# iPERDance/iPERCore

Hardware: AMD Instinct MI355X
Metric: synthesized frames/sec at 512x512 (run_imitator) (higher is better)
Workload: dtype f32; 1 GPU; run_imitator 512x512 single src/ref pair, 300-frame reference clip frame-sharded over 1 GPU(s), AttLWB-SPADE generator fp32 (BASELINE configs[1] at N = 1, configs[2] at N = 8); poses=imitate, image_size=512, frame_batch=300, frame_batch_requested=384, world_size=1, parallelism=frame-shard x1, batches_in_flight=1, weights=random-init (seeded) of the real architecture, 36,276,992 params

## Files before the change

### ipercore_amd/csrc/conv_winograd4.hip

```cpp
#include <hip/hip_runtime.h>
#include "lwg_common.h"
#include "lwg_conv_wino.h"

#define W4_THREADS 512
#define W4_PBX 8
#define W4_PBY 4
#define W4_NB 64
#define W4_KS 8
#define W4_HW 34
#define W4_HH 18
#ifndef W4_RS
#define W4_RS 40
#endif
#define W4_PLANE (18 * W4_RS + 4)
#define W4_RAW (W4_KS * W4_PLANE)
#define W4_VS (36 * W4_KS * 32)
#define W4_NEL (W4_HW * W4_HH * 2)
#define W4_NQ 3
#define W4_DUMP_OFF (2 * W4_RAW + 2 * W4_VS)
#define W4_DUMP (W4_THREADS + 3 * W4_PLANE)
#define W4_LOOP (W4_DUMP_OFF + W4_DUMP)
#define W4_MSR 68
#define W4_NPL 28
#define W4_MS (W4_NPL * 16 * W4_MSR)
#define W4_BIAS_OFF (W4_LOOP > W4_MS ? W4_LOOP : W4_MS)
#define W4F_SLOT(s) (((s) / CW4F_NSX) * CW4F_HH * W4_RS + ((s) % CW4F_NSX) * (W4_RS / CW4F_NSX))
#define W4F_PLANE (CW4F_NS / CW4F_NSX * CW4F_HH * W4_RS + 4)
static_assert(W4_RS / CW4F_NSX >= CW4F_HW && (W4_RS / CW4F_NSX) % 4 == 0 && W4F_PLANE >= W4_PLANE, "two sub-tile halo rows per LDS row");
#define W4F_LOOP (2 * W4_KS * W4F_PLANE + 2 * W4_VS + W4_THREADS + 3 * W4F_PLANE)
#define W4F_BIAS_OFF (W4F_LOOP > W4_MS ? W4F_LOOP : W4_MS)
static_assert(CW4F_SX == 16 && CW4F_SY == 8 && CW4F_NS * CW4F_ROUNDS * 64 == W4_NQ * W4_THREADS, "sub-tile halo: four slots x six wave rounds = the staged elements");
#ifndef LWG_W4_XCD
#define LWG_W4_XCD 1
#endif
#ifndef LWG_W4_CHUNK
#define LWG_W4_CHUNK 1
#endif
#ifndef LWG_W4_RDMAP
#define LWG_W4_RDMAP 1
#endif
#ifndef LWG_W4_SMALL
#define LWG_W4_SMALL 1
#endif
#define W4SB() __builtin_amdgcn_sched_barrier(0)

#ifdef LWG_W4_TS
#define W4TS(i) do { if (tid == 0 && lab_bi == 1) reinterpret_cast<unsigned long long*>(const_cast<float*>(a.res))[(size_t)blockIdx.x * 16 + (i)] = __builtin_readcyclecounter(); } while (0)
#define W4TSA(i) do { if (tid == 0) reinterpret_cast<unsigned long long*>(const_cast<float*>(a.res))[(size_t)blockIdx.x * 16 + (i)] = __builtin_readcyclecounter(); } while (0)
#else
#define W4TS(i) do { } while (0)
#define W4TSA(i) do { } while (0)
#endif

#ifndef W4_NT
#define W4_NT 0
#endif
#ifndef W4_NT_LD
#define W4_NT_LD W4_NT
#endif
#ifndef W4_NT_RES
#define W4_NT_RES 0
#endif
#ifndef W4_NT_ST
#define W4_NT_ST 2
#endif

__device__ __forceinline__ void w4_bt6(const float (&r)[6], float (&v)[6]) {
    const float a = __builtin_fmaf(-4.f, r[2], r[4]), b = __builtin_fmaf(-4.f, r[1], r[3]);
    const float c = r[4] - r[2], e = r[3] - r[1];
    v[0] = __builtin_fmaf(-5.f, r[2], __builtin_fmaf(4.f, r[0], r[4]));
    v[1] = a + b;
    v[2] = a - b;
    v[3] = __builtin_fmaf(2.f, e, c);
    v[4] = __builtin_fmaf(-2.f, e, c);
    v[5] = __builtin_fmaf(-5.f, r[3], __builtin_fmaf(4.f, r[1], r[5]));
}

__device__ __forceinline__ float w4_spade_mod(float x, float mu, float rs, float gam, float bet) { return (x - mu) * rs * (1.f + gam) + bet; }
template <int NR>
__device__ __forceinline__ void w4_act16(int act, floatx4 (&o)[NR]) {
    lwg_act_dispatch(act, [&](auto ACTC) {
        constexpr int EA = decltype(ACTC)::value;
#pragma unroll
        for (int i = 0; i < NR; ++i)
#pragma unroll
            for (int c = 0; c < 4; ++c) o[i][c] = lwg_act_c<EA>(o[i][c], act);
    });
}

template <int EPI, bool TWO, bool SM, bool LIST, bool FINE = false, bool SPLIT = false>
__device__ __forceinline__ void w4_body(const LwgConvArgs& a, const LwgConvLists& sk) {
    static_assert(!FINE || (LIST && !SM && !TWO && LWG_W4_RDMAP), "the sub-tile form: a list-driven 8-wave launch");
    static_assert(!SPLIT || (SM && !LIST && EPI == LWG_EPI_NONE), "the split form: 4-wave blocks, plain epilogue");
    constexpr int RS = W4_RS;
    constexpr int PLANE = FINE ? W4F_PLANE : W4_PLANE;
    constexpr int RAW = W4_KS * PLANE;
    constexpr int DUMP_OFF = 2 * RAW + 2 * W4_VS;
    constexpr int BIAS_OFF = FINE ? W4F_BIAS_OFF : W4_BIAS_OFF;
    constexpr bool SMS = SM && EPI == LWG_EPI_SPADE;
    constexpr int NVP = SM && !SMS ? 2 : 1;
    constexpr int NTH = SM ? 256 : W4_THREADS;
    constexpr int NQ = SM ? 5 : W4_NQ;
    constexpr int NBV = SM ? 32 : W4_NB;
    constexpr int MSR = SM ? 36 : W4_MSR;
    constexpr int NHF = SM ? 2 : 1;
    extern __shared__ __attribute__((aligned(16))) float smem[];
    const int wid = __builtin_amdgcn_readfirstlane(threadIdx.x >> 6);
    const float* __restrict__ bias = a.bias;
    const int H = a.H, W = a.W, Cin = a.C0 + a.C1, N = a.N;
    float* __restrict__ y = SPLIT ? a.y + cw4_slab_offset((int)blockIdx.z, a.M, N) : a.y;
    float* const raw0 = smem;
    float* const Ms = smem;
    const int tid = threadIdx.x, lane = tid & 63;
    const CwGrid g = cw_grid(a.B, H, W, N, 4 * W4_PBX, 4 * W4_PBY, NBV);
    const CwOrder o = cw_order(cw4_order_kind(LWG_W4_XCD, LWG_W4_CHUNK, SM, gridDim.x, N / NBV, Cin, N, g.tiles, g.total), gridDim.x, blockIdx.x, N / NBV, g);
    int blk = blockIdx.x;
    const int nall = FINE ? cw4f_in_image_total(a.B, H, W) : g.tiles;
    const int nht = LIST ? min(max(__builtin_amdgcn_readfirstlane(sk.counts[0]), 0), nall) : 0;
    const int nhe = (FINE ? cw4f_groups(nht) : nht) * (N / NBV);
    const bool lst = FINE ? true : LIST ? nht < nall : false;
    const bool run = lst ? blk < nhe : true;
    const int nst = Cin / W4_KS;
    const int sbeg = SPLIT ? cw4_slice_begin((int)blockIdx.z, a.cshift) : 0;
    const int send = SPLIT ? cw4_slice_end((int)blockIdx.z, a.cshift, nst) : nst;
    const __amdgpu_buffer_rsrc_t ru = __builtin_amdgcn_make_buffer_rsrc(const_cast<float*>(a.w), 0, (int)(144u * (unsigned)Cin * (unsigned)N), 0x00020000);
    const int q = wid & 3, ct = SM ? 0 : wid >> 2;
    const int half = SM ? 0 : wid >> 2;
    floatx16 acc[9];
    CwBlock<NQ, TWO> bk;
    unsigned uvoff, uvoffc;
    int fs0 = 0, fs1 = 0;
    auto setup = [&](int id) {
        int cb, t;
        if constexpr (FINE) {
            int tids = tid;
            asm volatile("" : "+v"(tids));
            int fsub[CW4F_NS], slot;
            cw_list_entry(id, N / NBV, slot, cb);
#pragma unroll
            for (int k = 0; k < CW4F_NS; ++k) {
                const int ix = cw4f_slot_index(slot, k, nht);
                fsub[k] = ix < 0 ? -1 : min(max(__builtin_amdgcn_readfirstlane(sk.heavy[ix]), 0), CW4F_NS * g.tiles - 1);
            }
            bk.n0 = cw_n0(cb, NBV);
            const int hs = wid >> 1, u = hs == 0 ? fsub[0] : hs == 1 ? fsub[1] : hs == 2 ? fsub[2] : fsub[3];
            int b, x0, y0;
            cw4f_corner(g, max(u, 0), b, x0, y0);
            bk.rx0 = cw_image_rsrc(a.x0, __builtin_amdgcn_readfirstlane(b), H, W, a.C0, 4u);
#pragma unroll
            for (int k = 0; k < NQ; ++k) {
                int s, j;
                cw4f_halo_elem(tids + NTH * k, s, j);
                bk.voff0[k] = cw4f_halo_voff(u >= 0, j, x0, y0, H, W, a.C0);
            }
            fs0 = (wid >> 2) ? fsub[1] : fsub[0], fs1 = (wid >> 2) ? fsub[CW4F_NSX + 1] : fsub[CW4F_NSX];
        } else if constexpr (LIST) {
            if (lst) {
                int slot;
                cw_list_entry(id, N / NBV, slot, cb);
                t = min(max(__builtin_amdgcn_readfirstlane(sk.heavy[slot]), 0), g.tiles - 1);
            } else {
                cw_block(o, id, cb, t);
            }
        } else {
            cw_block(o, id, cb, t);
        }
        if constexpr (!FINE) {
        bk.locate(a, g, t, 4 * W4_PBX, 4 * W4_PBY, SMS ? cw4_n0_spade_small(cb) : cw_n0(cb, NBV));
        int tids = tid;
        asm volatile("" : "+v"(tids));
        bk.halo(a, tids, NTH, W4_HW, W4_NEL);
        }
        const int col = SMS ? bk.n0 + (((lane & 31) >> 4) << 5) + (lane & 15) : bk.n0 + ct * 32 + (lane & 31);
        uvoff = (unsigned)(((lane >> 5) * 9 * N + 4 * col) * 4);
        uvoffc = (unsigned)(((lane >> 5) * 9 * N + 8 * N + col) * 4);
    };
    if (run) setup(blk);
    int wst[NQ];
#pragma unroll
    for (int k = 0; k < NQ; ++k) {
        const int i = tid + NTH * k;
        if constexpr (FINE) {
            int s, j, hy, hx, hq;
            cw4f_halo_elem(i, s, j);
            cw4f_halo_place(j, hy, hx, hq);
            wst[k] = j < CW4F_NEL ? 4 * hq * PLANE + W4F_SLOT(s) + hy * RS + hx : DUMP_OFF + tid;
        } else {
        const int pix = i >> 1, hq = i & 1, hy = pix / W4_HW, hx = pix - hy * W4_HW;
        wst[k] = i < W4_NEL ? 4 * hq * PLANE + hy * RS + hx : DUMP_OFF + tid;
        }
    }
    floatx4 rreg[NQ];
    auto rld1 = [&](int st, int k) -> floatx4 {
#ifdef W4_LAB_HFIX
        const int c = 0 * st;
#else
        const int c = st * W4_KS;
#endif
        return bk.template rld1<W4_NT_LD>(a, c, k);
    };
    auto rst1 = [&](int buf, int k, floatx4 v) { cw_rst1(raw0 + buf * RAW + wst[k], PLANE, v); };
    floatx4 ufa[4], ufb[4];
    float ufc[4];
    const unsigned ukk = (unsigned)N * 72u;
    const unsigned uq = (unsigned)q * (unsigned)nst * 4u * ukk;
    const unsigned ubo = (unsigned)N * 16u;
    auto uldpart = [&](int set, int st, int kk, int part) {
#ifdef W4_LAB_UFIX
        const unsigned so = uq + 0u * (unsigned)(st + kk);
#else
        const unsigned so = uq + (unsigned)(st * 4 + kk) * ukk;
#endif
        if (part == 0) ufa[set] = cw_buf_load(ru, uvoff, so);
        else if (part == 1) ufb[set] = cw_buf_load(ru, uvoff, so + ubo);
        else ufc[set] = __builtin_bit_cast(float, __builtin_amdgcn_raw_buffer_load_b32(ru, (int)uvoffc, (int)so, 0));
    };
    auto uldset = [&](int set, int st, int kk) {
#ifdef W4_LAB_UFIX
        const unsigned so = uq + 0u * (unsigned)(st + kk);
#else
        const unsigned so = uq + (unsigned)(st * 4 + kk) * ukk;
#endif
        ufa[set] = cw_buf_load(ru, uvoff, so);
        ufb[set] = cw_buf_load(ru, uvoff, so + ubo);
        ufc[set] = __builtin_bit_cast(float, __builtin_amdgcn_raw_buffer_load_b32(ru, (int)uvoffc, (int)so, 0));
    };
    const int patch = tid & 31, tc = (tid >> 5) & 7;
    const int pty = patch >> 3, ptx = patch & 7;
    int pby = pty, pbx = ptx, pslot = 0;
    if constexpr (FINE) {
        cw4f_patch_in_slot(pty, ptx, pby, pbx);
        pslot = W4F_SLOT(cw4f_slot_of_patch(pty, ptx));
    }
    unsigned dbs = (unsigned)(tc * PLANE + pslot + (4 * pby) * RS + 4 * pbx) >> 2;
    asm volatile("" : "+v"(dbs));
    dbs <<= 2;
    unsigned dbx[NHF], vbx[NHF], vbt[NHF];
    float alpha[NHF], beta[NHF], nbeta[NHF];
#pragma unroll
    for (int hi = 0; hi < NHF; ++hi) {
        const int hf = SM ? hi : half;
        dbx[hi] = (unsigned)(tc * PLANE + pslot + (4 * pby + hf) * RS + 4 * pbx) >> 2;
        asm volatile("" : "+v"(dbx[hi]));
        dbx[hi] <<= 2;
        vbx[hi] = (unsigned)(2 * RAW + (hf ? 30 : 0) * W4_KS * 32 + tc * 32 + patch);
        vbt[hi] = (unsigned)(2 * RAW + (hf ? 18 : 6) * W4_KS * 32 + tc * 32 + patch);
        asm volatile("" : "+v"(vbx[hi]));
        asm volatile("" : "+v"(vbt[hi]));
        alpha[hi] = hf ? -1.f : -4.f;
        beta[hi] = hf ? 2.f : 1.f;
        nbeta[hi] = -beta[hi];
    }
    unsigned fbs[2];
    fbs[0] = (unsigned)(2 * RAW + (6 * q) * W4_KS * 32 + lane);
    fbs[1] = (unsigned)(2 * RAW + (6 * (4 + (q >> 1)) + 3 * (q & 1)) * W4_KS * 32 + lane);
    asm volatile("" : "+v"(fbs[0]));
    asm volatile("" : "+v"(fbs[1]));
    float fb[9];
    auto frag1 = [&](int buf, int kk, int j) -> float {
        return smem[fbs[j < 6 ? 0 : 1] + buf * W4_VS + ((j < 6 ? j : j - 6) * W4_KS + 2 * kk) * 32];
// ... 99 lines not shown
                    vst6(vbt[hi], set ^ 1, step - 12, v);
                }
            }
            W4SB();
        };
        if constexpr (!SM) {
            mf(0, 0, true); ul(0, 0);
            mf(0, 1, true); halo(0);
            mf(0, 2, true); ul(0, 1); tr(0, 0);
            mf(0, 3, true); halo(1); tr(0, 1);
            mf(0, 4, true); ul(0, 2); tr(0, 2);
            mf(0, 5, true); halo(2);
            mf(0, 6, true); tr(0, 3);
            mf(0, 7, true); tr(0, 4);
            mf(0, 8, true); tr(0, 5);
            mf(1, 0, true); ul(1, 0); tr(0, 6);
            mf(1, 1, true); tr(0, 7);
            mf(1, 2, true); ul(1, 1); tr(0, 8); tr(0, 9);
            mf(1, 3, true); tr(0, 10);
            mf(1, 4, true); ul(1, 2);
            mf(1, 5, true); tr(0, 11);
            mf(1, 6, true); tr(0, 12);
            mf(1, 7, true);
            mf(1, 8, true); tr(0, 13);
            mf(2, 0, true); ul(2, 0);
            mf(2, 1, true);
            mf(2, 2, true); ul(2, 1);
            mf(2, 3, true);
            mf(2, 4, true); ul(2, 2);
            mf(2, 5, true); mf(2, 6, true); mf(2, 7, true); mf(2, 8, true);
        } else {
            mf(0, 0, true); ul(0, 0); halo(0);
            mf(0, 1, true); tr(0, 0);
            mf(0, 2, true); ul(0, 1); tr(0, 1);
            mf(0, 3, true); halo(1); tr(0, 2);
            mf(0, 4, true); ul(0, 2); tr(0, 3);
            mf(0, 5, true); halo(2); tr(0, 4);
            mf(0, 6, true); tr(0, 5);
            mf(0, 7, true); halo(3); tr(0, 6);
            mf(0, 8, true); tr(0, 7);
            mf(1, 0, true); ul(1, 0); tr(0, 8); tr(0, 9);
            mf(1, 1, true); halo(4); tr(0, 10);
            mf(1, 2, true); ul(1, 1); tr(0, 11);
            mf(1, 3, true); tr(0, 12);
            mf(1, 4, true); ul(1, 2); tr(0, 13);
            mf(1, 5, true); tr(1, 0);
            mf(1, 6, true); tr(1, 1);
            mf(1, 7, true); tr(1, 2);
            mf(1, 8, true); tr(1, 3);
            mf(2, 0, true); ul(2, 0); tr(1, 4);
            mf(2, 1, true); tr(1, 5);
            mf(2, 2, true); ul(2, 1); tr(1, 6);
            mf(2, 3, true); tr(1, 7);
            mf(2, 4, true); ul(2, 2); tr(1, 8); tr(1, 9);
            mf(2, 5, true); tr(1, 10);
            mf(2, 6, true); tr(1, 11);
            mf(2, 7, true); tr(1, 12);
            mf(2, 8, true); tr(1, 13);
        }
        __syncthreads();
        W4SB();
        mf(3, 0, nxt); ul(3, 0);
        mf(3, 1, nxt);
        mf(3, 2, nxt); ul(3, 1);
        mf(3, 3, nxt);
        mf(3, 4, nxt); ul(3, 2);
        mf(3, 5, nxt); mf(3, 6, nxt); mf(3, 7, nxt); mf(3, 8, nxt);
    };

    floatx4 r0[NQ], r1[NQ];
    float bq;
    auto issue_loads = [&]() {
        bq = bias ? bias[SMS ? bk.n0 + (((tid & 31) >> 4) << 5) + (tid & 15) : bk.n0 + (tid & (NBV - 1))] : 0.f;
#pragma unroll
        for (int k = 0; k < NQ; ++k) {
            r0[k] = rld1(sbeg, k);
            r1[k] = rld1(sbeg + 1, k);
        }
        uldset(0, sbeg, 0);
        uldset(1, sbeg, 1);
#pragma unroll
        for (int k = 0; k < NQ; ++k) rreg[k] = rld1(send - sbeg > 2 ? sbeg + 2 : sbeg + 1, k);
    };
    if (run) issue_loads();
#ifdef LWG_W4_TS
    int lab_bi = 0;
#endif
    W4TSA(11);
    if (run) for (;;) {
    W4TS(0);
#pragma unroll
    for (int k = 0; k < NQ; ++k) {
        rst1(0, k, r0[k]);
        rst1(1, k, r1[k]);
    }
    if (tid < NBV) smem[BIAS_OFF + tid] = bq;
    __syncthreads();
    transform_full(0);
    __syncthreads();
#pragma unroll
    for (int j = 0; j < 9; ++j) fb[j] = frag1(0, 0, j);
#pragma unroll
    for (int j = 0; j < 9; ++j)
#pragma unroll
        for (int r = 0; r < 16; ++r) acc[j][r] = 0.f;
    if (q == 1) {
#pragma unroll
        for (int g = 0; g < 4; ++g) {
            const floatx4 b4 = *reinterpret_cast<const floatx4*>(smem + BIAS_OFF + ct * 32 + 8 * g + 4 * (lane >> 5));
#pragma unroll
            for (int k = 0; k < 4; ++k) acc[1][4 * g + k] = b4[k];
        }
    }
    W4TS(1);
    {
        int s = sbeg;
        for (; s + 2 < send; s += 2) {
            iteration(s, IntC<0>(), IntC<1>());
            iteration(s + 1, IntC<1>(), IntC<1>());
        }
        iteration(s, IntC<0>(), IntC<1>());
        iteration(s + 1, IntC<1>(), IntC<0>());
    }
    W4TS(2);
    int eb = FINE ? 0 : bk.b, ex0 = FINE ? 0 : bk.x0, ey0 = FINE ? 0 : bk.y0;
    const int en0 = bk.n0;
    const int es0 = fs0, es1 = fs1;
#pragma unroll
    for (int r = 0; r < 16; ++r) {
        const float m0 = acc[0][r], m1 = acc[1][r], m2 = acc[2][r], m3 = acc[3][r], m4 = acc[4][r], m5 = acc[5][r];
        const float s12 = m1 + m2, d12 = m1 - m2, s34 = m3 + m4, d34 = m3 - m4;
        acc[0][r] = (m0 + s12) + s34;
        acc[1][r] = __builtin_fmaf(2.f, d34, d12);
        acc[2][r] = __builtin_fmaf(4.f, s34, s12);
        acc[3][r] = __builtin_fmaf(8.f, d34, d12) + m5;
    }
    if (q & 1) {
#pragma unroll
        for (int r = 0; r < 16; ++r) {
            const float h0 = acc[6][r], h1 = acc[7][r];
            acc[6][r] = h0 + h1;
            acc[7][r] = h0 - h1;
        }
    } else {
#pragma unroll
        for (int r = 0; r < 16; ++r) {
            const float h0 = acc[6][r], h1 = acc[7][r], h2 = acc[8][r];
            acc[6][r] = (h0 + h1) + h2;
            acc[7][r] = h1 - h2;
            acc[8][r] = h1 + h2;
        }
    }
    W4TS(4);
    int tide = tid;
    asm volatile("" : "+v"(tide));
    const int lanee = tide & 63;
    const int rb = wid & 3;
    const unsigned l5 = (unsigned)lanee & 31u, gsel = (0x0FF0F00Fu >> l5) & 1u;
    const int gidx = __builtin_popcount((gsel ? 0x0FF0F00Fu : 0xF00F0FF0u) & ((1u << l5) - 1u));
    const int p16 = LWG_W4_RDMAP && !SM ? (wid >> 2) * 4 + 2 * (lanee >> 5) + (gsel ? 0 : 1) + 8 * (gidx >> 3) : (wid >> 2) * 8 + (lanee >> 3);
    const int n4 = SMS ? (lanee & 3) * 4 : LWG_W4_RDMAP && !SM ? (gidx & 7) * 4 : (lanee & 7) * 4;
    const int cbase = SMS ? (en0 >> 6) * 32 + ((en0 >> 4) & 1) * 16 : en0 >> 1;
    floatx4 mu, rs;
    typedef unsigned int w4_u4 __attribute__((ext_vector_type(4)));
    const unsigned img_bytes = (unsigned)(H * W) * (unsigned)a.YC * 4u;
    const float* const esrc = EPI == LWG_EPI_SPADE ? a.xn : EPI == LWG_EPI_RESIDUAL ? a.res : a.y;
    __amdgpu_buffer_rsrc_t ry, re;
    auto eframe = [&]() {
        if (EPI == LWG_EPI_SPADE) {
            mu = *reinterpret_cast<const floatx4*>(a.mean + (size_t)eb * a.YC + cbase + n4);
            rs = *reinterpret_cast<const floatx4*>(a.rstd + (size_t)eb * a.YC + cbase + n4);
        }
        ry = __builtin_amdgcn_make_buffer_rsrc(y + (size_t)eb * H * W * a.YC, 0, (int)img_bytes, 0x00020000);
        re = __builtin_amdgcn_make_buffer_rsrc(const_cast<float*>(esrc) + (size_t)eb * H * W * a.YC, 0, (int)img_bytes, 0x00020000);
    };
    if constexpr (!FINE) eframe();
    const int chan = EPI == LWG_EPI_SPADE ? cbase + n4 : a.ycoff + en0 + n4;
    bool more = false;
    int nblk = blk;
#pragma unroll
    for (int ph = 0; ph < 2; ++ph) {
        if (ph == 1) __syncthreads();
        if constexpr (FINE) {
            const int u = ph ? es1 : es0;
            int ub;
            cw4f_corner(g, max(u, 0), ub, ex0, ey0);
            eb = __builtin_amdgcn_readfirstlane(ub);
            if (u < 0) ex0 = W, ey0 = H;
            eframe();
        }
        if (((lanee >> 4) & 1) == ph) {
            float* dst = Ms + (lanee & 15) * MSR + ct * 32 + 4 * (lanee >> 5);
#pragma unroll
            for (int g = 0; g < 4; ++g) {
#pragma unroll
                for (int bb = 0; bb < 4; ++bb)
                    *reinterpret_cast<floatx4*>(dst + (4 * q + bb) * 16 * MSR + 8 * g) = floatx4{acc[bb][4 * g], acc[bb][4 * g + 1], acc[bb][4 * g + 2], acc[bb][4 * g + 3]};
#pragma unroll
                for (int i = 0; i < 3; ++i)
                    *reinterpret_cast<floatx4*>(dst + (16 + 3 * q + i) * 16 * MSR + 8 * g) = floatx4{acc[6 + i][4 * g], acc[6 + i][4 * g + 1], acc[6 + i][4 * g + 2], acc[6 + i][4 * g + 3]};
            }
        }
        unsigned vo[NVP][4];
#pragma unroll
        for (int hp = 0; hp < NVP; ++hp) {
            const int p = ph * 16 + (SMS ? lanee >> 2 : SM ? 8 * hp + (lanee >> 3) : p16);
            const int ox = ex0 + 4 * (FINE ? (p & 7) % (CW4F_SX / 4) : (p & 7)) + rb, oyb = ey0 + 4 * (FINE ? (p >> 3) % (CW4F_SY / 4) : (p >> 3));
#pragma unroll
            for (int i = 0; i < 4; ++i)
                vo[hp][i] = cw4_out_voff(ox, oyb + i, H, W, a.YC, chan);
        }
        floatx4 ext[2][4];
        if (EPI != LWG_EPI_NONE) {
#pragma unroll
            for (int h = 0; h < (EPI == LWG_EPI_SPADE ? 1 : 2); ++h)
#pragma unroll
                for (int i = 0; i < 4; ++i) ext[h][i] = __builtin_bit_cast(floatx4, __builtin_amdgcn_raw_buffer_load_b128(re, (int)cw4_out_group(vo[NVP == 2 ? h : 0][i], h, !SM), 0, W4_NT_RES));
        }
        if (ph == 1) {
            W4TS(8);
            if constexpr (!SPLIT) {
            nblk = blk + (int)gridDim.x;
            if constexpr (FINE) more = nblk < nhe;
            else if constexpr (LIST) more = lst ? nblk < nhe : cw_has_block(o, nblk);
            else more = cw_has_block(o, nblk);
            setup(more ? nblk : blk);
            W4TS(9);
            issue_loads();
            W4TS(10);
            }
        }
        __syncthreads();
        if (ph == 0) W4TS(5); else W4TS(7);
        floatx4 gam[4];
#pragma unroll
        for (int h = 0; h < 2; ++h) {
            const float* base = Ms + (SMS ? lanee >> 2 : SM ? 8 * h + (lanee >> 3) : p16) * MSR + (SMS ? h * 16 : SM ? 0 : h * 32) + n4;
            floatx4 F[6];
#pragma unroll
            for (int xi = 0; xi < 4; ++xi) F[xi] = *reinterpret_cast<const floatx4*>(base + (4 * xi + rb) * 16 * MSR);
            const int ia = rb == 0 ? 0 : rb == 2 ? 2 : 1, ib = (rb & 1) ? 4 : 3;
            const float cb = (float)(1 << rb);
#pragma unroll
            for (int r = 0; r < 2; ++r) {
                const float* hb = base + (16 + 6 * r) * 16 * MSR;
                const floatx4 pa = *reinterpret_cast<const floatx4*>(hb + ia * 16 * MSR);
                const floatx4 pb = *reinterpret_cast<const floatx4*>(hb + ib * 16 * MSR);
                floatx4 f;
#pragma unroll
                for (int c = 0; c < 4; ++c) f[c] = __builtin_fmaf(cb, pb[c], pa[c]);
                if (rb == 3) f += *reinterpret_cast<const floatx4*>(hb + 5 * 16 * MSR);
                F[4 + r] = f;
            }
            floatx4 o[4];
#pragma unroll
            for (int c = 0; c < 4; ++c) {
                const float s12 = F[1][c] + F[2][c], d12 = F[1][c] - F[2][c], s34 = F[3][c] + F[4][c], d34 = F[3][c] - F[4][c];
                o[0][c] = (F[0][c] + s12) + s34;
                o[1][c] = __builtin_fmaf(2.f, d34, d12);
                o[2][c] = __builtin_fmaf(4.f, s34, s12);
                o[3][c] = __builtin_fmaf(8.f, d34, d12) + F[5][c];
            }
            if (EPI == LWG_EPI_SPADE) {
                if (h == 0) {
#pragma unroll
                    for (int i = 0; i < 4; ++i) gam[i] = o[i];
                    continue;
                }
#pragma unroll
                for (int i = 0; i < 4; ++i)
#pragma unroll
                    for (int c = 0; c < 4; ++c) o[i][c] = w4_spade_mod(ext[0][i][c], mu[c], rs[c], gam[i][c], o[i][c]);
            } else if (EPI == LWG_EPI_RESIDUAL) {
                if (a.act == LWG_ACT_RELU_MASK) {
#pragma unroll
                    for (int i = 0; i < 4; ++i)
#pragma unroll
                        for (int c = 0; c < 4; ++c) o[i][c] = ext[h][i][c] > 0.f ? o[i][c] : 0.f;
                } else {
#pragma unroll
                    for (int i = 0; i < 4; ++i) o[i] += ext[h][i];
                }
            }
            w4_act16(a.act, o);
#pragma unroll
            for (int i = 0; i < 4; ++i)
                __builtin_amdgcn_raw_buffer_store_b128(__builtin_bit_cast(w4_u4, o[i]), ry, (int)cw4_out_group(vo[NVP == 2 ? h : 0][i], h, EPI != LWG_EPI_SPADE && !SM), 0, W4_NT_ST);
        }
        if (ph == 0) W4TS(6);
    }
    W4TS(3);
#ifdef LWG_W4_TS
    ++lab_bi;
#endif
    if (!more) break;
    blk = nblk;
    __syncthreads();
    }
    W4TSA(12);
#ifdef LWG_W4_TS
    if (tid == 0) reinterpret_cast<unsigned long long*>(const_cast<float*>(a.res))[(size_t)blockIdx.x * 16 + 13] = (unsigned long long)lab_bi;
#endif
    if constexpr (LIST) {
        typedef unsigned int w4_u4 __attribute__((ext_vector_type(4)));
        constexpr int NQD = EPI == LWG_EPI_SPADE ? 8 : 16;
        constexpr int NPASS = (FINE ? CW4F_SX * CW4F_SY : 512) * NQD / W4_THREADS, NI = NPASS < 4 ? NPASS : 4;
        const int ncb = N / NBV;
        const int nend = nhe + min(max(__builtin_amdgcn_readfirstlane(sk.counts[1]), 0), nall - nht) * ncb;
        const unsigned img_bytes = (unsigned)(H * W) * (unsigned)a.YC * 4u;
        const __amdgpu_buffer_rsrc_t rc = __builtin_amdgcn_make_buffer_rsrc(const_cast<float*>(sk.cal), 0, (int)((unsigned)(H * W) * (unsigned)(EPI == LWG_EPI_SPADE ? N : a.YC) * 4u), 0x00020000);
#pragma unroll 1
        for (int id = cw_list_first_light((int)blockIdx.x, (int)gridDim.x, nhe); id < nend; id += (int)gridDim.x) {
            int slot, cb;
            cw_list_entry(id - nhe, ncb, slot, cb);
            const int t = min(max(__builtin_amdgcn_readfirstlane(sk.light[slot]), 0), (FINE ? CW4F_NS : 1) * g.tiles - 1);
            const int en0 = cw_n0(cb, NBV);
            int eb, ex0, ey0;
            if constexpr (FINE) {
                cw4f_corner(g, t, eb, ex0, ey0);
                eb = __builtin_amdgcn_readfirstlane(eb);
            } else {
                eb = __builtin_amdgcn_readfirstlane(cw_image(g, t));
                cw_corner(g, t - eb * g.bx * g.by, 4 * W4_PBX, 4 * W4_PBY, ex0, ey0);
            }
            const __amdgpu_buffer_rsrc_t ry = __builtin_amdgcn_make_buffer_rsrc(y + (size_t)eb * H * W * a.YC, 0, (int)img_bytes, 0x00020000);
            int px, py, q4;
            cw4_light_elem(tid, 0, W4_THREADS, NQD, px, py, q4);
            if constexpr (EPI == LWG_EPI_SPADE) {
                const __amdgpu_buffer_rsrc_t re = __builtin_amdgcn_make_buffer_rsrc(const_cast<float*>(a.xn) + (size_t)eb * H * W * a.YC, 0, (int)img_bytes, 0x00020000);
                const int cbase = en0 >> 1;
                const floatx4 mu = *reinterpret_cast<const floatx4*>(a.mean + (size_t)eb * a.YC + cbase + 4 * q4);
                const floatx4 rs = *reinterpret_cast<const floatx4*>(a.rstd + (size_t)eb * a.YC + cbase + 4 * q4);
#pragma unroll 1
                for (int it = 0; it < NPASS; it += NI) {
                    unsigned vo[NI];
                    floatx4 o[NI], gam[NI], xv[NI];
#pragma unroll
                    for (int i = 0; i < NI; ++i) {
                        cw4_light_elem(tid, it + i, W4_THREADS, NQD, px, py, q4);
                        if constexpr (FINE) cw4f_light_pixel(px, py);
                        vo[i] = cw4_out_voff(ex0 + px, ey0 + py, H, W, a.YC, cbase + 4 * q4);
                        const unsigned vc = cw4_out_voff(ex0 + px, ey0 + py, H, W, N, en0 + 4 * q4);
                        gam[i] = cw_buf_load(rc, cw4_out_group(vc, 0, true), 0u);
                        o[i] = cw_buf_load(rc, cw4_out_group(vc, 1, true), 0u);
                        xv[i] = cw_buf_load<W4_NT_RES>(re, vo[i], 0u);
                    }
#pragma unroll
                    for (int i = 0; i < NI; ++i)
#pragma unroll
                        for (int c = 0; c < 4; ++c) o[i][c] = w4_spade_mod(xv[i][c], mu[c], rs[c], gam[i][c], o[i][c]);
                    w4_act16(a.act, o);
#pragma unroll
                    for (int i = 0; i < NI; ++i) __builtin_amdgcn_raw_buffer_store_b128(__builtin_bit_cast(w4_u4, o[i]), ry, (int)vo[i], 0, W4_NT_ST);
                }
            } else {
#pragma unroll 1
                for (int it = 0; it < NPASS; it += NI) {
                    unsigned vo[NI];
                    floatx4 o[NI];
#pragma unroll
                    for (int i = 0; i < NI; ++i) {
                        cw4_light_elem(tid, it + i, W4_THREADS, NQD, px, py, q4);
                        if constexpr (FINE) cw4f_light_pixel(px, py);
                        vo[i] = cw4_out_voff(ex0 + px, ey0 + py, H, W, a.YC, a.ycoff + en0 + 4 * q4);
                        o[i] = cw_buf_load(rc, vo[i], 0u);
                    }
#pragma unroll
                    for (int i = 0; i < NI; ++i) __builtin_amdgcn_raw_buffer_store_b128(__builtin_bit_cast(w4_u4, o[i]), ry, (int)vo[i], 0, W4_NT_ST);
                }
            }
        }
    }
}

template <int EPI, bool TWO, bool SM = false>
__global__ __launch_bounds__(SM ? 256 : W4_THREADS, 1) void lwg_conv_winograd4_kernel(const LwgConvArgs a) {
    w4_body<EPI, TWO, SM, false>(a, LwgConvLists{});
}
template <bool TWO>
__global__ __launch_bounds__(256, 1) void lwg_conv_winograd4_split_kernel(const LwgConvArgs a) {
    w4_body<LWG_EPI_NONE, TWO, true, false, false, true>(a, LwgConvLists{});
}
template <int EPI>
__global__ __launch_bounds__(W4_THREADS, 1) void lwg_conv_winograd4_list_kernel(const LwgConvArgs a, const LwgConvLists sk) {
    w4_body<EPI, false, false, true>(a, sk);
}
template <int EPI>
__global__ __launch_bounds__(W4_THREADS, 1) void lwg_conv_winograd4_fine_kernel(const LwgConvArgs a, const LwgConvLists sk) {
    if (__builtin_amdgcn_readfirstlane(sk.counts[0]) >= cw4f_in_image_total(a.B, a.H, a.W)) return;
    w4_body<EPI, false, false, true, true>(a, sk);
}
template <int EPI>
__global__ __launch_bounds__(W4_THREADS, 1) void lwg_conv_winograd4_fine_plain_kernel(const LwgConvArgs a, const LwgConvLists sk) {
    if (__builtin_amdgcn_readfirstlane(sk.counts[0]) < cw4f_in_image_total(a.B, a.H, a.W)) return;
    w4_body<EPI, false, false, false>(a, LwgConvLists{});
}


__global__ __launch_bounds__(256) void lwg_winograd4_panel_kernel(const float* __restrict__ wp, float* __restrict__ U, int Cin, int N, LwgWinoTaps taps) {
    const int n = blockIdx.x * 64 + (threadIdx.x & 63), c = blockIdx.y * 4 + (threadIdx.x >> 6);
    if (n >= N || c >= Cin) return;
    double g[3][3];
#pragma unroll
    for (int r = 0; r < 3; ++r)
#pragma unroll
        for (int s = 0; s < 3; ++s) {
            const int k = ((c >> 5) * 9 + taps.t[3 * r + s]) * 32 + (c & 31);
            g[r][s] = (double)wp[((size_t)(k >> 2) * N + n) * 4 + (k & 3)];
        }
    const double G[6][3] = {{1.0 / 4, 0, 0}, {-1.0 / 6, -1.0 / 6, -1.0 / 6}, {-1.0 / 6, 1.0 / 6, -1.0 / 6}, {1.0 / 24, 1.0 / 12, 1.0 / 6}, {1.0 / 24, -1.0 / 12, 1.0 / 6}, {0, 0, 1}};
    double t[6][3];
#pragma unroll
    for (int i = 0; i < 6; ++i)
#pragma unroll
        for (int s = 0; s < 3; ++s) t[i][s] = G[i][0] * g[0][s] + G[i][1] * g[1][s] + G[i][2] * g[2][s];
    const int s8 = c >> 3, kk = (c & 7) >> 1, kh = c & 1;
#pragma unroll
    for (int qq = 0; qq < 4; ++qq) {
        float* dst = U + ((((size_t)qq * (Cin >> 3) + s8) * 4 + kk) * 2 + kh) * 9 * (size_t)N;
        float o[9];
#pragma unroll
        for (int j = 0; j < 9; ++j) {
            const int xi = j < 6 ? qq : 4 + (qq >> 1), nu = j < 6 ? j : 3 * (qq & 1) + (j - 6);
            o[j] = (float)(t[xi][0] * G[nu][0] + t[xi][1] * G[nu][1] + t[xi][2] * G[nu][2]);
        }
        *reinterpret_cast<floatx4*>(dst + 4 * n) = floatx4{o[0], o[1], o[2], o[3]};
        *reinterpret_cast<floatx4*>(dst + 4 * (size_t)N + 4 * n) = floatx4{o[4], o[5], o[6], o[7]};
        dst[8 * (size_t)N + n] = o[8];
    }
}

__device__ __forceinline__ double w4_panel_sum3(double a0, double b0, double a1, double b1, double a2, double b2) {
#pragma clang fp contract(off)
    const double p = a0 * b0;
    return __builtin_fma(a2, b2, __builtin_fma(a1, b1, p));
}
__device__ __forceinline__ void lwg_winograd4_panels_pair(const float* __restrict__ wp, float* __restrict__ U, int Cin, int N, const int* t9, int c, int n) {
    double g[3][3];
#pragma unroll
    for (int r = 0; r < 3; ++r)
#pragma unroll
        for (int s = 0; s < 3; ++s) {
            const int k = ((c >> 5) * 9 + t9[3 * r + s]) * 32 + (c & 31);
            g[r][s] = (double)wp[((size_t)(k >> 2) * N + n) * 4 + (k & 3)];
        }
    const double G[6][3] = {{1.0 / 4, 0, 0}, {-1.0 / 6, -1.0 / 6, -1.0 / 6}, {-1.0 / 6, 1.0 / 6, -1.0 / 6}, {1.0 / 24, 1.0 / 12, 1.0 / 6}, {1.0 / 24, -1.0 / 12, 1.0 / 6}, {0, 0, 1}};
    double t[6][3];
#pragma unroll
    for (int i = 0; i < 6; ++i)
#pragma unroll
        for (int s = 0; s < 3; ++s) t[i][s] = w4_panel_sum3(G[i][0], g[0][s], G[i][1], g[1][s], G[i][2], g[2][s]);
    const int s8 = c >> 3, kk = (c & 7) >> 1, kh = c & 1;
#pragma unroll
    for (int qq = 0; qq < 4; ++qq) {
        float* dst = U + ((((size_t)qq * (Cin >> 3) + s8) * 4 + kk) * 2 + kh) * 9 * (size_t)N;
// ... 137 lines not shown
```

### ipercore_amd/csrc/lwg_conv_wino.h

```cpp
#pragma once
#include <stddef.h>
#include "lwg_conv_args.h"

#ifdef __HIPCC__
#define CW_FN __host__ __device__ __forceinline__
#else
#define CW_FN static inline
#endif
#ifdef __HIP_DEVICE_COMPILE__
#define CW_UNIFORM(v) __builtin_amdgcn_readfirstlane(v)
#else
#define CW_UNIFORM(v) (v)
#endif
#define CW_OOB 0xC0000000u
#define CW_KS 8
#define CW_NB 64
struct CwGrid { int bx, by, tiles, total; };
CW_FN CwGrid cw_grid(int B, int H, int W, int N, int ex, int ey, int nbv) {
    const int bx = (W + ex - 1) / ex, by = (H + ey - 1) / ey, tiles = bx * by * B;
    return CwGrid{bx, by, tiles, tiles * (N / nbv)};
}
CW_FN long long cw_total_blocks(int B, int H, int W, int N, int ex, int ey, int nbv) {
    return (long long)((W + ex - 1) / ex) * ((H + ey - 1) / ey) * B * (N / nbv);
}

enum { CW_COLMAJOR = 0, CW_CHUNK = 1, CW_XCD = 2 };
struct CwOrder { int kind, nwg, wg, ncb, tiles, total, xg, xr; };

CW_FN int cw4_order_kind(int xcd_sw, int chunk_sw, bool sm, unsigned nwg, int ncb, int Cin, int N, int tiles, int total) {
    const bool xcd = xcd_sw && !sm && (nwg & 7u) == 0 && (ncb == 4 || ncb == 8 || (ncb == 2 && (Cin >= 192 || xcd_sw == 2))) && (int)nwg < total && tiles >= (int)nwg / ncb;
    return xcd ? CW_XCD : chunk_sw == 2 || (chunk_sw == 1 && 144u * (unsigned)Cin * (unsigned)N <= (5u << 20)) ? CW_CHUNK : CW_COLMAJOR;
}
CW_FN CwOrder cw_order(int kind, unsigned nwg, unsigned wg, int ncb, const CwGrid& g) {
    return CwOrder{kind, (int)nwg, (int)wg, ncb, g.tiles, g.total, (int)nwg / ncb, (int)(((wg & 7u) / (unsigned)ncb) * (nwg >> 3) + (wg >> 3))};
}
CW_FN bool cw_has_block(const CwOrder& o, int id) {
    return o.kind == CW_XCD ? (id / o.nwg) * o.xg + o.xr < o.tiles : id < o.total;
}
CW_FN void cw_block(const CwOrder& o, int id, int& cb, int& t) {
    if (o.kind == CW_XCD) {
        cb = (int)((unsigned)o.wg & 7u) & (o.ncb - 1);
        t = CW_UNIFORM((id / o.nwg) * o.xg + o.xr);
    } else if (o.kind == CW_CHUNK) {
        const int G = o.nwg, per = G * o.ncb;
        const int ch = CW_UNIFORM(id / per);
        const int r = id - ch * per, base = ch * G;
        const int nt = o.tiles - base < G ? o.tiles - base : G;
        cb = CW_UNIFORM(r / nt);
        t = CW_UNIFORM(base + r - cb * nt);
    } else {
        cb = CW_UNIFORM(id / o.tiles);
        t = CW_UNIFORM(id - cb * o.tiles);
    }
}
CW_FN int cw_image(const CwGrid& g, int t) { return t / (g.bx * g.by); }
CW_FN void cw_corner(const CwGrid& g, int t_in_image, int ex, int ey, int& x0, int& y0) { x0 = (t_in_image % g.bx) * ex, y0 = (t_in_image / g.bx) * ey; }
CW_FN int cw_n0(int cb, int nbv) { return cb * nbv; }
CW_FN int cw4_n0_spade_small(int cb) { return (cb >> 1) * 64 + (cb & 1) * 16; }
CW_FN int cw_halo_pixel(int i, int hw, int nel, int lgp, int x0, int y0, int H, int W) {
    const int pix = i >> lgp, hy = pix / hw, hx = pix - hy * hw;
    const int gy = y0 - 1 + hy, gx = x0 - 1 + hx;
    return i < nel && gy >= 0 && gy < H && gx >= 0 && gx < W ? gy * W + gx : -1;
}
CW_FN unsigned cw_halo_pixel_voff(int lin, int i, int lgp, int C, int ebytes) {
    return lin >= 0 ? (unsigned)(lin * C + (16 / ebytes) * (i & ((1 << lgp) - 1))) * (unsigned)ebytes : CW_OOB;
}
CW_FN unsigned cw_halo_voff(int i, int hw, int nel, int lgp, int x0, int y0, int H, int W, int C, int ebytes) {
    return cw_halo_pixel_voff(cw_halo_pixel(i, hw, nel, lgp, x0, y0, H, W), i, lgp, C, ebytes);
}
CW_FN bool cw_stage_second(int c, int C0, bool two) { return two && c >= C0; }
CW_FN unsigned cw_stage_soff(int c, int C0, bool two, int ebytes) { return (unsigned)(cw_stage_second(c, C0, two) ? c - C0 : c) * (unsigned)ebytes; }
CW_FN unsigned cw4_out_voff(int ox, int oy, int H, int W, int YC, int chan) {
    return ox < W && oy < H ? (unsigned)((oy * W + ox) * YC + chan) * 4u : CW_OOB;
}
CW_FN unsigned cw4_out_group(unsigned vo, int h, bool grouped) { return vo + (grouped ? 128u * (unsigned)h : 0u); }

struct CwWindow { int x0, y0, x1, y1; };
CW_FN CwWindow cw_block_window(int x0, int y0, int ex, int ey, int d, int H, int W) {
    return CwWindow{x0 - d > 0 ? x0 - d : 0, y0 - d > 0 ? y0 - d : 0, x0 + ex + d < W ? x0 + ex + d : W, y0 + ey + d < H ? y0 + ey + d : H};
}
CW_FN void cw_list_entry(int e, int ncb, int& slot, int& cb) { slot = e / ncb, cb = e - slot * ncb; }
CW_FN int cw_list_first_light(int wg, int nwg, int nhe) { return wg >= nhe ? wg : wg + (nhe - wg + nwg - 1) / nwg * nwg; }
CW_FN void cw4_light_elem(int tid, int it, int nth, int nq, int& px, int& py, int& q4) {
    const int e = it * nth + tid, p = e / nq;
    q4 = e - p * nq, px = p & 31, py = p >> 5;
}

#define CW4F_SX 16
#define CW4F_SY 8
#define CW4F_NSX (32 / CW4F_SX)
#define CW4F_NS (CW4F_NSX * (16 / CW4F_SY))
#define CW4F_HW (CW4F_SX + 2)
#define CW4F_HH (CW4F_SY + 2)
#define CW4F_NEL (CW4F_HW * CW4F_HH * 2)
#define CW4F_ROUNDS ((CW4F_NEL + 63) / 64)
CW_FN int cw4f_slot_of_patch(int pty, int ptx) { return (pty / (CW4F_SY / 4)) * CW4F_NSX + ptx / (CW4F_SX / 4); }
CW_FN void cw4f_patch_in_slot(int pty, int ptx, int& ly, int& lx) { ly = pty % (CW4F_SY / 4), lx = ptx % (CW4F_SX / 4); }
CW_FN void cw4f_corner(const CwGrid& g, int u, int& b, int& x0, int& y0) {
    const int t = u / CW4F_NS, s = u - t * CW4F_NS;
    b = cw_image(g, t);
    cw_corner(g, t - b * g.bx * g.by, 32, 16, x0, y0);
    x0 += (s % CW4F_NSX) * CW4F_SX, y0 += (s / CW4F_NSX) * CW4F_SY;
}
CW_FN bool cw4f_in_image(int x0, int y0, int H, int W) { return x0 < W && y0 < H; }
CW_FN int cw4f_in_image_total(int B, int H, int W) { return B * ((W + CW4F_SX - 1) / CW4F_SX) * ((H + CW4F_SY - 1) / CW4F_SY); }
CW_FN int cw4f_groups(int nh) { return (nh + CW4F_NS - 1) / CW4F_NS; }
CW_FN int cw4f_slot_index(int grp, int k, int nh) { return grp * CW4F_NS + k < nh ? grp * CW4F_NS + k : -1; }
CW_FN unsigned cw4f_reached(int x, int y, int x0, int y0, int d) {
    unsigned m = 0;
    for (int s = 0; s < CW4F_NS; ++s) {
        const int sx = x0 + (s % CW4F_NSX) * CW4F_SX, sy = y0 + (s / CW4F_NSX) * CW4F_SY;
        m |= (x >= sx - d && x < sx + CW4F_SX + d && y >= sy - d && y < sy + CW4F_SY + d ? 1u : 0u) << s;
    }
    return m;
}
CW_FN void cw4f_halo_elem(int i, int& slot, int& j) {
    const int wave = (i >> 6) & 7, k = i >> 9, per = CW4F_ROUNDS / 3, wr = 3 * wave + k;
    slot = wave / per, j = (wr - slot * CW4F_ROUNDS) * 64 + (i & 63);
}
CW_FN void cw4f_halo_place(int j, int& hy, int& hx, int& hq) {
    const int pix = j >> 1;
    hq = j & 1, hy = pix / CW4F_HW, hx = pix - hy * CW4F_HW;
}
CW_FN unsigned cw4f_halo_voff(bool present, int j, int x0, int y0, int H, int W, int C) {
    int hy, hx, hq;
    cw4f_halo_place(j, hy, hx, hq);
    const int gy = y0 - 1 + hy, gx = x0 - 1 + hx;
    return present && j < CW4F_NEL && gy >= 0 && gy < H && gx >= 0 && gx < W ? (unsigned)((gy * W + gx) * C + 4 * hq) * 4u : CW_OOB;
}
CW_FN void cw4f_light_pixel(int& px, int& py) {
    const int p = py * 32 + px;
    py = p / CW4F_SX, px = p - py * CW4F_SX;
}

#define CW4_SPLIT_MIN_STAGES 8
#define CW4_SPLIT_MAX_SLICES 8
struct Cw4Split { int slices, sps; };
CW_FN Cw4Split cw4_split_plan(long long blocks32, int nst, int cus, bool finishable, bool slab_ok) {
    if (!finishable || !slab_ok || blocks32 < 1 || 2 * blocks32 > (long long)cus) return Cw4Split{0, 0};
    int want = (int)((long long)cus / blocks32);
    if (want > CW4_SPLIT_MAX_SLICES) want = CW4_SPLIT_MAX_SLICES;
    int sps = (nst + want - 1) / want;
    if (sps < CW4_SPLIT_MIN_STAGES) sps = CW4_SPLIT_MIN_STAGES;
    sps += sps & 1;
    const int slices = (nst + sps - 1) / sps;
    return slices < 2 ? Cw4Split{0, 0} : Cw4Split{slices, sps};
}
CW_FN int cw4_slice_begin(int slice, int sps) { return slice * sps; }
CW_FN int cw4_slice_end(int slice, int sps, int nst) { return (slice + 1) * sps < nst ? (slice + 1) * sps : nst; }
CW_FN size_t cw4_slab_offset(int slice, int M, int N) { return (size_t)slice * (size_t)M * (size_t)N; }
CW_FN bool cw4_slab_image_ok(int H, int W, int N) { return (unsigned long long)H * W * N * 4ull + 256ull < (unsigned long long)CW_OOB; }

#define CW_NO_OUT_BUFFER (-1ll)
CW_FN bool cw_contract_ok(const LwgConvArgs& a, unsigned long long pair_bytes, long long out_slack) {
    if (!a.x0 || !a.w || !a.y || a.M <= 0 || a.ntaps != 9 || a.stride != 1 || a.omul != 1 || a.C0 <= 0 || (a.C0 % CW_KS) != 0 || a.C1 < 0 ||
        (a.C1 % CW_KS) != 0 || ((a.C0 + a.C1) % (2 * CW_KS)) != 0 || (a.C1 > 0 && !a.x1) || a.N <= 0 || (a.N % CW_NB) != 0 || a.OH != a.H ||
        a.OW != a.W || a.YH != a.H || a.YW != a.W || a.xdt != LWG_DT_F32 || a.ydt != LWG_DT_F32 || (long long)a.M != (long long)a.B * a.H * a.W ||
        a.ycoff < 0 || (a.ycoff % 4) != 0 || (a.YC % 4) != 0 || (a.act == LWG_ACTIVATION_RELU_MASK && a.epi != LWG_EPI_RESIDUAL))
        return false;
    if (a.epi == LWG_EPI_SPADE) {
        if (!a.xn || !a.mean || !a.rstd || !a.bias || a.YC * 2 != a.N || a.ycoff != 0) return false;
    } else {
        if (a.ycoff + a.N > a.YC) return false;
        if (a.epi != LWG_EPI_NONE && (a.epi != LWG_EPI_RESIDUAL || !a.res)) return false;
    }
// ... 102 lines not shown
```

Baseline: 1362 frames/s.

## Stagger light-tile copy pass across heavy-tile iterations in list Winograd conv

Measured after the change: 1372 frames/s (median of 6 runs). About the same (+0.7%).

```diff
diff --git a/ipercore_amd/csrc/conv_winograd4.hip b/ipercore_amd/csrc/conv_winograd4.hip
--- a/ipercore_amd/csrc/conv_winograd4.hip
+++ b/ipercore_amd/csrc/conv_winograd4.hip
@@ -41,6 +41,9 @@
 #endif
 #ifndef LWG_W4_SMALL
 #define LWG_W4_SMALL 1
+#endif
+#ifndef LWG_W4_STAGGER
+#define LWG_W4_STAGGER 32
 #endif
 #define W4SB() __builtin_amdgcn_sched_barrier(0)
 
@@ -120,6 +123,9 @@
     const int nhe = (FINE ? cw4f_groups(nht) : nht) * (N / NBV);
     const bool lst = FINE ? true : LIST ? nht < nall : false;
     const bool run = lst ? blk < nhe : true;
+    constexpr bool STAG = LIST && LWG_W4_STAGGER > 1;
+    const int lat = STAG && lst ? cw_list_light_at((int)blockIdx.x, (int)gridDim.x, nhe, LWG_W4_STAGGER) : -1;
+    bool srun = run, pro = true;
     const int nst = Cin / W4_KS;
     const int sbeg = SPLIT ? cw4_slice_begin((int)blockIdx.z, a.cshift) : 0;
     const int send = SPLIT ? cw4_slice_end((int)blockIdx.z, a.cshift, nst) : nst;
@@ -175,7 +181,7 @@
         uvoff = (unsigned)(((lane >> 5) * 9 * N + 4 * col) * 4);
         uvoffc = (unsigned)(((lane >> 5) * 9 * N + 8 * N + col) * 4);
     };
-    if (run) setup(blk);
+    if constexpr (!STAG) { if (run) setup(blk); }
     int wst[NQ];
 #pragma unroll
     for (int k = 0; k < NQ; ++k) {
@@ -441,12 +447,95 @@
 #pragma unroll
         for (int k = 0; k < NQ; ++k) rreg[k] = rld1(send - sbeg > 2 ? sbeg + 2 : sbeg + 1, k);
     };
-    if (run) issue_loads();
+    if constexpr (!STAG) { if (run) issue_loads(); }
 #ifdef LWG_W4_TS
     int lab_bi = 0;
 #endif
     W4TSA(11);
-    if (run) for (;;) {
+    auto light = [&]() {
+    if constexpr (LIST) {
+        typedef unsigned int w4_u4 __attribute__((ext_vector_type(4)));
+        constexpr int NQD = EPI == LWG_EPI_SPADE ? 8 : 16;
+        constexpr int NPASS = (FINE ? CW4F_SX * CW4F_SY : 512) * NQD / W4_THREADS, NI = NPASS < 4 ? NPASS : 4;
+        const int ncb = N / NBV;
+        const int nend = nhe + min(max(__builtin_amdgcn_readfirstlane(sk.counts[1]), 0), nall - nht) * ncb;
+        const unsigned img_bytes = (unsigned)(H * W) * (unsigned)a.YC * 4u;
+        const __amdgpu_buffer_rsrc_t rc = __builtin_amdgcn_make_buffer_rsrc(const_cast<float*>(sk.cal), 0, (int)((unsigned)(H * W) * (unsigned)(EPI == LWG_EPI_SPADE ? N : a.YC) * 4u), 0x00020000);
+        int tidl = tid;
+        if constexpr (STAG) asm volatile("" : "+v"(tidl));
+        const int tid = tidl;
+#pragma unroll 1
+        for (int id = cw_list_first_light((int)blockIdx.x, (int)gridDim.x, nhe); id < nend; id += (int)gridDim.x) {
+            int slot, cb;
+            cw_list_entry(id - nhe, ncb, slot, cb);
+            const int t = min(max(__builtin_amdgcn_readfirstlane(sk.light[slot]), 0), (FINE ? CW4F_NS : 1) * g.tiles - 1);
+            const int en0 = cw_n0(cb, NBV);
+            int eb, ex0, ey0;
+            if constexpr (FINE) {
+                cw4f_corner(g, t, eb, ex0, ey0);
+                eb = __builtin_amdgcn_readfirstlane(eb);
+            } else {
+                eb = __builtin_amdgcn_readfirstlane(cw_image(g, t));
+                cw_corner(g, t - eb * g.bx * g.by, 4 * W4_PBX, 4 * W4_PBY, ex0, ey0);
+            }
+            const __amdgpu_buffer_rsrc_t ry = __builtin_amdgcn_make_buffer_rsrc(y + (size_t)eb * H * W * a.YC, 0, (int)img_bytes, 0x00020000);
+            int px, py, q4;
+            cw4_light_elem(tid, 0, W4_THREADS, NQD, px, py, q4);
+            if constexpr (EPI == LWG_EPI_SPADE) {
+                const __amdgpu_buffer_rsrc_t re = __builtin_amdgcn_make_buffer_rsrc(const_cast<float*>(a.xn) + (size_t)eb * H * W * a.YC, 0, (int)img_bytes, 0x00020000);
+                const int cbase = en0 >> 1;
+                const floatx4 mu = *reinterpret_cast<const floatx4*>(a.mean + (size_t)eb * a.YC + cbase + 4 * q4);
+                const floatx4 rs = *reinterpret_cast<const floatx4*>(a.rstd + (size_t)eb * a.YC + cbase + 4 * q4);
+#pragma unroll 1
+                for (int it = 0; it < NPASS; it += NI) {
+                    unsigned vo[NI];
+                    floatx4 o[NI], gam[NI], xv[NI];
+#pragma unroll
+                    for (int i = 0; i < NI; ++i) {
+                        cw4_light_elem(tid, it + i, W4_THREADS, NQD, px, py, q4);
+                        if constexpr (FINE) cw4f_light_pixel(px, py);
+                        vo[i] = cw4_out_voff(ex0 + px, ey0 + py, H, W, a.YC, cbase + 4 * q4);
+                        const unsigned vc = cw4_out_voff(ex0 + px, ey0 + py, H, W, N, en0 + 4 * q4);
+                        gam[i] = cw_buf_load(rc, cw4_out_group(vc, 0, true), 0u);
+                        o[i] = cw_buf_load(rc, cw4_out_group(vc, 1, true), 0u);
+                        xv[i] = cw_buf_load<W4_NT_RES>(re, vo[i], 0u);
+                    }
+#pragma unroll
+                    for (int i = 0; i < NI; ++i)
+#pragma unroll
+                        for (int c = 0; c < 4; ++c) o[i][c] = w4_spade_mod(xv[i][c], mu[c], rs[c], gam[i][c], o[i][c]);
+                    w4_act16(a.act, o);
+#pragma unroll
+                    for (int i = 0; i < NI; ++i) __builtin_amdgcn_raw_buffer_store_b128(__builtin_bit_cast(w4_u4, o[i]), ry, (int)vo[i], 0, W4_NT_ST);
+                }
+            } else {
+#pragma unroll 1
+                for (int it = 0; it < NPASS; it += NI) {
+                    unsigned vo[NI];
+                    floatx4 o[NI];
+#pragma unroll
+                    for (int i = 0; i < NI; ++i) {
+                        cw4_light_elem(tid, it + i, W4_THREADS, NQD, px, py, q4);
+                        if constexpr (FINE) cw4f_light_pixel(px, py);
+                        vo[i] = cw4_out_voff(ex0 + px, ey0 + py, H, W, a.YC, a.ycoff + en0 + 4 * q4);
+                        o[i] = cw_buf_load(rc, vo[i], 0u);
+                    }
+#pragma unroll
+                    for (int i = 0; i < NI; ++i) __builtin_amdgcn_raw_buffer_store_b128(__builtin_bit_cast(w4_u4, o[i]), ry, (int)vo[i], 0, W4_NT_ST);
+                }
+            }
+        }
+    }
+    };
+    if (STAG || run) for (;;) {
+    if constexpr (STAG) {
+        if (pro) {
+            if (blk == lat) light();
+            if (!srun) break;
+            setup(blk);
+            issue_loads();
+        }
+    }
     W4TS(0);
 #pragma unroll
     for (int k = 0; k < NQ; ++k) {
@@ -583,7 +672,8 @@
             if constexpr (FINE) more = nblk < nhe;
             else if constexpr (LIST) more = lst ? nblk < nhe : cw_has_block(o, nblk);
             else more = cw_has_block(o, nblk);
-            setup(more ? nblk : blk);
+            if constexpr (STAG) pro = !more || nblk == lat;
+            setup(STAG ? (pro ? blk : nblk) : more ? nblk : blk);
             W4TS(9);
             issue_loads();
             W4TS(10);
@@ -652,7 +742,11 @@
 #ifdef LWG_W4_TS
     ++lab_bi;
 #endif
+    if constexpr (STAG) {
+        srun = more;
+    } else {
     if (!more) break;
+    }
     blk = nblk;
     __syncthreads();
     }
@@ -660,76 +754,7 @@
 #ifdef LWG_W4_TS
     if (tid == 0) reinterpret_cast<unsigned long long*>(const_cast<float*>(a.res))[(size_t)blockIdx.x * 16 + 13] = (unsigned long long)lab_bi;
 #endif
-    if constexpr (LIST) {
-        typedef unsigned int w4_u4 __attribute__((ext_vector_type(4)));
-        constexpr int NQD = EPI == LWG_EPI_SPADE ? 8 : 16;
-        constexpr int NPASS = (FINE ? CW4F_SX * CW4F_SY : 512) * NQD / W4_THREADS, NI = NPASS < 4 ? NPASS : 4;
-        const int ncb = N / NBV;
-        const int nend = nhe + min(max(__builtin_amdgcn_readfirstlane(sk.counts[1]), 0), nall - nht) * ncb;
-        const unsigned img_bytes = (unsigned)(H * W) * (unsigned)a.YC * 4u;
-        const __amdgpu_buffer_rsrc_t rc = __builtin_amdgcn_make_buffer_rsrc(const_cast<float*>(sk.cal), 0, (int)((unsigned)(H * W) * (unsigned)(EPI == LWG_EPI_SPADE ? N : a.YC) * 4u), 0x00020000);
-#pragma unroll 1
-        for (int id = cw_list_first_light((int)blockIdx.x, (int)gridDim.x, nhe); id < nend; id += (int)gridDim.x) {
-            int slot, cb;
-            cw_list_entry(id - nhe, ncb, slot, cb);
-            const int t = min(max(__builtin_amdgcn_readfirstlane(sk.light[slot]), 0), (FINE ? CW4F_NS : 1) * g.tiles - 1);
-            const int en0 = cw_n0(cb, NBV);
-            int eb, ex0, ey0;
-            if constexpr (FINE) {
-                cw4f_corner(g, t, eb, ex0, ey0);
-                eb = __builtin_amdgcn_readfirstlane(eb);
-            } else {
-                eb = __builtin_amdgcn_readfirstlane(cw_image(g, t));
-                cw_corner(g, t - eb * g.bx * g.by, 4 * W4_PBX, 4 * W4_PBY, ex0, ey0);
-            }
-            const __amdgpu_buffer_rsrc_t ry = __builtin_amdgcn_make_buffer_rsrc(y + (size_t)eb * H * W * a.YC, 0, (int)img_bytes, 0x00020000);
-            int px, py, q4;
-            cw4_light_elem(tid, 0, W4_THREADS, NQD, px, py, q4);
-            if constexpr (EPI == LWG_EPI_SPADE) {
-                const __amdgpu_buffer_rsrc_t re = __builtin_amdgcn_make_buffer_rsrc(const_cast<float*>(a.xn) + (size_t)eb * H * W * a.YC, 0, (int)img_bytes, 0x00020000);
-                const int cbase = en0 >> 1;
-                const floatx4 mu = *reinterpret_cast<const floatx4*>(a.mean + (size_t)eb * a.YC + cbase + 4 * q4);
-                const floatx4 rs = *reinterpret_cast<const floatx4*>(a.rstd + (size_t)eb * a.YC + cbase + 4 * q4);
-#pragma unroll 1
-                for (int it = 0; it < NPASS; it += NI) {
-                    unsigned vo[NI];
-                    floatx4 o[NI], gam[NI], xv[NI];
-#pragma unroll
-                    for (int i = 0; i < NI; ++i) {
-                        cw4_light_elem(tid, it + i, W4_THREADS, NQD, px, py, q4);
-                        if constexpr (FINE) cw4f_light_pixel(px, py);
-                        vo[i] = cw4_out_voff(ex0 + px, ey0 + py, H, W, a.YC, cbase + 4 * q4);
-                        const unsigned vc = cw4_out_voff(ex0 + px, ey0 + py, H, W, N, en0 + 4 * q4);
-                        gam[i] = cw_buf_load(rc, cw4_out_group(vc, 0, true), 0u);
-                        o[i] = cw_buf_load(rc, cw4_out_group(vc, 1, true), 0u);
-                        xv[i] = cw_buf_load<W4_NT_RES>(re, vo[i], 0u);
-                    }
-#pragma unroll
-                    for (int i = 0; i < NI; ++i)
-#pragma unroll
-                        for (int c = 0; c < 4; ++c) o[i][c] = w4_spade_mod(xv[i][c], mu[c], rs[c], gam[i][c], o[i][c]);
-                    w4_act16(a.act, o);
-#pragma unroll
-                    for (int i = 0; i < NI; ++i) __builtin_amdgcn_raw_buffer_store_b128(__builtin_bit_cast(w4_u4, o[i]), ry, (int)vo[i], 0, W4_NT_ST);
-                }
-            } else {
-#pragma unroll 1
-                for (int it = 0; it < NPASS; it += NI) {
-                    unsigned vo[NI];
-                    floatx4 o[NI];
-#pragma unroll
-                    for (int i = 0; i < NI; ++i) {
-                        cw4_light_elem(tid, it + i, W4_THREADS, NQD, px, py, q4);
-                        if constexpr (FINE) cw4f_light_pixel(px, py);
-                        vo[i] = cw4_out_voff(ex0 + px, ey0 + py, H, W, a.YC, a.ycoff + en0 + 4 * q4);
-                        o[i] = cw_buf_load(rc, vo[i], 0u);
-                    }
-#pragma unroll
-                    for (int i = 0; i < NI; ++i) __builtin_amdgcn_raw_buffer_store_b128(__builtin_bit_cast(w4_u4, o[i]), ry, (int)vo[i], 0, W4_NT_ST);
-                }
-            }
-        }
-    }
+    if constexpr (LIST && !STAG) light();
 }
 
 template <int EPI, bool TWO, bool SM = false>
diff --git a/ipercore_amd/csrc/lwg_conv_wino.h b/ipercore_amd/csrc/lwg_conv_wino.h
--- a/ipercore_amd/csrc/lwg_conv_wino.h
+++ b/ipercore_amd/csrc/lwg_conv_wino.h
@@ -81,6 +81,14 @@
 }
 CW_FN void cw_list_entry(int e, int ncb, int& slot, int& cb) { slot = e / ncb, cb = e - slot * ncb; }
 CW_FN int cw_list_first_light(int wg, int nwg, int nhe) { return wg >= nhe ? wg : wg + (nhe - wg + nwg - 1) / nwg * nwg; }
+#define CW_STAGGER_RUN 8
+CW_FN int cw_list_heavy_count(int wg, int nwg, int nhe) { return wg >= nhe ? 0 : (nhe - wg + nwg - 1) / nwg; }
+CW_FN int cw_list_phase(int wg, int phases) { return phases > 1 ? (wg / CW_STAGGER_RUN) % phases : 0; }
+CW_FN int cw_list_stagger(int wg, int nwg, int nhe, int phases) {
+    const int hc = cw_list_heavy_count(wg, nwg, nhe), p1 = cw_list_phase(wg, phases) + 1;
+    return phases > 1 ? hc / phases * p1 + hc % phases * p1 / phases : hc;
+}
+CW_FN int cw_list_light_at(int wg, int nwg, int nhe, int phases) { return wg + cw_list_stagger(wg, nwg, nhe, phases) * nwg; }
 CW_FN void cw4_light_elem(int tid, int it, int nth, int nq, int& px, int& py, int& q4) {
     const int e = it * nth + tid, p = e / nq;
     q4 = e - p * nq, px = p & 31, py = p >> 5;
```
